# HKUST-Aerial-Robotics/FIESTA

Measured on AMD Instinct MI355X. Metric: esdf_updated_voxels_per_sec, higher is better.
Workload: dtype u32

## Files before the change

fiesta_amd/csrc/dense_map.hip:

```cpp
#include "dense_map.hpp"
#include "checkpoint.hpp"
#include "frontier_kernels.hpp"
#include "ray_query_kernels.hpp"
#include "reach_kernels.hpp"
#include "reach_path_kernels.hpp"
#include "cluster_kernels.hpp"
#include "view_kernels.hpp"
#include "ft_kernels.hpp"
#include "nn_kernels.hpp"
#include "mask_kernels.hpp"
#include "level_kernels.hpp"
#include "path_cost_kernels.hpp"
#include "path_kernels.hpp"
#include "relax_kernels.hpp"

#include <algorithm>
#include <chrono>
#include <cmath>
#include <cstdlib>
#include <cstring>

namespace fiesta {

template <typename T>
// ... 830 lines not shown
  ntiles_ = ntx_ * nty_ * ntz_;

  FIESTA_HIP_CHECK(hipStreamCreateWithFlags(&stream_, hipStreamNonBlocking));
  FIESTA_HIP_CHECK(hipEventCreate(&ev0_));
  FIESTA_HIP_CHECK(hipEventCreate(&ev1_));
  FIESTA_HIP_CHECK(hipMalloc((void **)&coc_, g.n * sizeof(vox_t)));
  FIESTA_HIP_CHECK(hipMalloc((void **)&logodds_, g.n * sizeof(double)));
  FIESTA_HIP_CHECK(hipMalloc((void **)&cnt_, g.n * sizeof(unsigned long long)));
  FIESTA_HIP_CHECK(hipMalloc((void **)&occbits_, nbitwords_ * sizeof(uint32_t)));
  FIESTA_HIP_CHECK(hipMalloc((void **)&rbits_, nbitwords_ * sizeof(uint32_t)));
  FIESTA_HIP_CHECK(hipMalloc((void **)&obsbits_, nbitwords_ * sizeof(uint32_t)));
  FIESTA_HIP_CHECK(hipMalloc((void **)&latebits_, nbitwords_ * sizeof(uint32_t)));
  FIESTA_HIP_CHECK(hipMemsetAsync(obsbits_, 0, nbitwords_ * sizeof(uint32_t), stream_));
  FIESTA_HIP_CHECK(hipMemsetAsync(latebits_, 0, nbitwords_ * sizeof(uint32_t), stream_));
  if (sharded) {
    ngoccwords_ = (int64_t)g.GX * g.GY * g.GZW;
    FIESTA_HIP_CHECK(hipMalloc((void **)&gocc_, ngoccwords_ * sizeof(uint32_t)));
    FIESTA_HIP_CHECK(hipMemsetAsync(gocc_, 0, ngoccwords_ * sizeof(uint32_t), stream_));
  }
  FIESTA_HIP_CHECK(hipMalloc((void **)&tile_epoch_, ntiles_ * sizeof(uint32_t)));
  for (int k = 0; k < 2; ++k) {
    FIESTA_HIP_CHECK(hipMalloc((void **)&cbits_[k], nbitwords_ * sizeof(uint32_t)));
    FIESTA_HIP_CHECK(hipMalloc((void **)&cstamp_[k], ntiles_ * sizeof(uint32_t)));
    FIESTA_HIP_CHECK(hipMemsetAsync(cbits_[k], 0, nbitwords_ * sizeof(uint32_t), stream_));
    FIESTA_HIP_CHECK(hipMemsetAsync(cstamp_[k], 0, ntiles_ * sizeof(uint32_t), stream_));
  }
  for (int k = 0; k < 2; ++k) {
    FIESTA_HIP_CHECK(hipMalloc((void **)&tile_flag_[k], ntiles_ * sizeof(uint32_t)));
    FIESTA_HIP_CHECK(hipMalloc((void **)&tile_list_[k], ntiles_ * sizeof(uint32_t)));
    FIESTA_HIP_CHECK(hipMemsetAsync(tile_flag_[k], 0, ntiles_ * sizeof(uint32_t), stream_));
  }
  FIESTA_HIP_CHECK(hipMalloc((void **)&counters_, C_COUNT * sizeof(unsigned long long)));
  FIESTA_HIP_CHECK(hipHostMalloc((void **)&h_counters_, C_COUNT * sizeof(unsigned long long)));
  FIESTA_HIP_CHECK(hipMemsetAsync(counters_, 0, C_COUNT * sizeof(unsigned long long), stream_));
  hipLaunchKernelGGL(k_fill<vox_t>, dim3(grid_for(g.n, 256, 4096)), dim3(256), 0, stream_, coc_, kUnobserved, g.n);
  FIESTA_HIP_CHECK(hipGetLastError());
  FIESTA_HIP_CHECK(hipMemsetAsync(logodds_, 0, g.n * sizeof(double), stream_));
  FIESTA_HIP_CHECK(hipMemsetAsync(cnt_, 0, g.n * sizeof(unsigned long long), stream_));
  FIESTA_HIP_CHECK(hipMemsetAsync(occbits_, 0, nbitwords_ * sizeof(uint32_t), stream_));
  FIESTA_HIP_CHECK(hipMemsetAsync(rbits_, 0, nbitwords_ * sizeof(uint32_t), stream_));
  FIESTA_HIP_CHECK(hipMemsetAsync(tile_epoch_, 0, ntiles_ * sizeof(uint32_t), stream_));
  set_original_range();
  pp_ = ProbParams{0, 0, 0, 0, 0};
#ifdef FIESTA_HIP_TUNING
  if (const char *e = getenv("FIESTA_HIP_PROF")) prof_ = atoi(e);
  if (const char *e = getenv("FIESTA_HIP_SPATIAL")) spatial_ = atoi(e);
  if (const char *e = getenv("FIESTA_HIP_LIST_THRESHOLD")) list_threshold_ = std::max(0, atoi(e));
  if (const char *e = getenv("FIESTA_HIP_SMALL_UPDATE")) small_update_ = std::max(0, atoi(e));
  if (const char *e = getenv("FIESTA_HIP_BOUND_SCAN")) bound_scan_ = atoi(e);
  if (const char *e = getenv("FIESTA_HIP_BLOCKS")) spatial_blocks_ = std::max(8, atoi(e) / 8 * 8);
  if (const char *e = getenv("FIESTA_HIP_BULK_RATIO")) bulk_ratio_ = atof(e);
  if (const char *e = getenv("FIESTA_HIP_FT_S0")) ft_s0_ = atoi(e);
#endif
  if (ft_s0_ != 16 && ft_s0_ != 32) throw Error(FIESTA_HIP_ERR_INVALID, "FIESTA_HIP_FT_S0 must be 16 or 32");
  for (auto &e : ft_ev_) FIESTA_HIP_CHECK(hipEventCreate(&e));
  FIESTA_HIP_CHECK(hipStreamSynchronize(stream_));
}

DenseMap::~DenseMap() {
  (void)hipSetDevice(device_);
  if (stream_) (void)hipStreamSynchronize(stream_);
  free_raycast_state();
  void *ptrs[] = {coc_,          logodds_,      cnt_,          occbits_,      rbits_,     tile_epoch_,
                  tile_flag_[0], tile_flag_[1], tile_list_[0], tile_list_[1], counters_,  cbits_[0],
                  cbits_[1],     cstamp_[0],    cstamp_[1],    gocc_,         obsbits_,   latebits_,
                  mask_ctr_};
  for (void *p : ptrs)
    if (p) (void)hipFree(p);
  if (h_counters_) (void)hipHostFree(h_counters_);
  if (h_mask_ctr_) (void)hipHostFree(h_mask_ctr_);
  delete bricks_;
  delete lv_;
  for (hipEvent_t e : evpool_) (void)hipEventDestroy(e);
  for (hipEvent_t e : ft_ev_)
    if (e) (void)hipEventDestroy(e);
  if (ev0_) (void)hipEventDestroy(ev0_);
  if (ev1_) (void)hipEventDestroy(ev1_);
  if (stream_) (void)hipStreamDestroy(stream_);
}

void DenseMap::set_prob_params(double p_hit, double p_miss, double p_min, double p_max, double p_occ) {
  auto logit = [](double x) { return std::log(x / (1 - x)); };
  pp_.l_hit = logit(p_hit);
  pp_.l_miss = logit(p_miss);
  pp_.l_min = logit(p_min);
  pp_.l_max = logit(p_max);
  pp_.l_occ = logit(p_occ);
}

void DenseMap::set_original_range() {
  Geom &g = g_;
  g.wx0 = g.wy0 = g.wz0 = 0;
  g.wx1 = g.nx - 1;
  g.wy1 = g.ny - 1;
  g.wz1 = g.nz - 1;
  g.px0 = g.wx0, g.py0 = g.wy0, g.pz0 = g.wz0;
  g.px1 = g.wx1, g.py1 = g.wy1, g.pz1 = g.wz1;
}

void DenseMap::set_update_range(const double *mn, const double *mx, bool new_vec) {
  Geom &g = g_;
  double a[3], b[3];
  for (int i = 0; i < 3; ++i) {
    a[i] = std::max(mn[i], g.lo[i]);
    b[i] = std::min(mx[i], g.hi[i]);
  }
// ... 459 lines not shown
  a.ticket = &counters_[C_FUSE_TICKET];
  if (!g.sharded && !a.g.big()) {
    a.fail_cap = (uint32_t)std::min<int64_t>(std::max<int64_t>(ncells / 64, 16), 4096);
    nn_fail_list_.ensure((size_t)a.fail_cap, stream_);
    a.fail_list = nn_fail_list_.p, a.nfail = &counters_[C_NN_BRUTE];
    if (publish && !incremental) a.nsparse = &counters_[C_NN_SPARSE];
  }
  const unsigned close_blocks = nn_last_brute_ > 0 ? (unsigned)std::min<long long>(nn_last_brute_ + 8, 512) : 1u;
  a.cursor = &counters_[C_NN_CURSOR], a.failed = &counters_[C_NN_FAILED], a.entries = &counters_[C_NN_ENTRIES];
  const bool want_max = (track_ && !tr_out_) || open_side;
  a.maxd2 = want_max ? &counters_[C_FT_MAXD2] : nullptr;
  ft_in_place_ = !g.sharded || (!open_side && alone_in_group_);
  if (!ft_in_place_) ft_out_.ensure_exact((size_t)g.n, stream_);
  a.coc = tr_out_ ? tr_out_ : ft_in_place_ ? coc_ : ft_out_.p;
  if (publish) {
    a.pub = h_counters_, a.queues = &counters_[C_INSERT], a.track_dst = track_ ? &counters_[C_MAXD2] : nullptr;
    a.tag = ++nn_tag_;
    a.pub_failed = C_NN_FAILED, a.pub_entries = C_NN_ENTRIES, a.pub_maxd2 = C_FT_MAXD2, a.pub_tag = C_NN_CURSOR, a.pub_dirty = C_NN_DIRTY;
    a.pub_brute = C_NN_BRUTE, a.pub_sparse = C_NN_SPARSE;
  }
  if (!ft_counters_clean_)
    FIESTA_HIP_CHECK(hipMemsetAsync(&counters_[C_FT_OVF0], 0, 7 * sizeof(unsigned long long), stream_));
  ft_counters_clean_ = false;
  FIESTA_HIP_CHECK(hipEventRecord(ft_ev_[0], stream_));
  if (a.szb % 4 == 0) hipLaunchKernelGGL(k_nn_cells<true>, dim3((unsigned)((nrows + 15) / 16)), dim3(1024), 0, stream_, a);
  else hipLaunchKernelGGL(k_nn_cells<false>, dim3((unsigned)((nrows + 15) / 16)), dim3(1024), 0, stream_, a);
  FIESTA_HIP_CHECK(hipGetLastError());
  FIESTA_HIP_CHECK(hipEventRecord(ft_ev_[1], stream_));
  const int lcx = a.g.lx1 - a.g.lx0, lcy = a.g.ly1 - a.g.ly0, lcz = a.g.lz1 - a.g.lz0;
  if (incremental) {
    hipLaunchKernelGGL(k_nn_mark, dim3((unsigned)std::min<unsigned long long>((ni + nd) * 3375 / 1024 + 1, 256)), dim3(1024), 0, stream_, a);
    const unsigned est = (unsigned)std::min<unsigned long long>((ni + nd) * 200 + 256, (unsigned long long)ncells / 2);
    hipLaunchKernelGGL(k_nn_lists_dirty, dim3(std::min(std::max(est / 16u, 64u), 8192u)), dim3(256), 0, stream_, a);
    FIESTA_HIP_CHECK(hipGetLastError());
    FIESTA_HIP_CHECK(hipEventRecord(ft_ev_[2], stream_));
    if (want_max) hipLaunchKernelGGL(k_nn_fill_dirty<true>, dim3(std::min(std::max(est / 4u, 64u), 8192u)), dim3(256), 0, stream_, a);
    else hipLaunchKernelGGL(k_nn_fill_dirty<false>, dim3(std::min(std::max(est / 4u, 64u), 8192u)), dim3(256), 0, stream_, a);
    FIESTA_HIP_CHECK(hipGetLastError());
    FIESTA_HIP_CHECK(hipEventRecord(ft_ev_[3], stream_));
    if (publish) {
      NnArgs c = a;
      c.nfail = nullptr, c.nsparse = nullptr;
      hipLaunchKernelGGL(k_nn_close, dim3(1), dim3(256), 0, stream_, c);
      FIESTA_HIP_CHECK(hipGetLastError());
    }
    if (st) {
      st->bulk = 1;
      st->cells = 1;
      st->nn_incremental = 1;
      st->relax_launches = 4;
    }
    return true;
  }
  if (a.g.big()) hipLaunchKernelGGL(k_nn_lists<true>, dim3((lcz + 63) / 64, (lcy + 3) / 4, lcx), dim3(1024), 0, stream_, a);
  else hipLaunchKernelGGL(k_nn_lists<false>, dim3((lcz + 63) / 64, (lcy + 3) / 4, lcx), dim3(1024), 0, stream_, a);
  FIESTA_HIP_CHECK(hipGetLastError());
  FIESTA_HIP_CHECK(hipEventRecord(ft_ev_[2], stream_));
  const int64_t nq = nrows * ((a.g.ncz + 3) / 4);
  unsigned fill_blocks = 0;
  bool full = (a.g.fx | a.g.fy | a.g.fz) == 0 && a.g.nx == g.nx && a.g.ny == g.ny && a.g.nz == g.nz && g.nx % nn::kB == 0 &&
              g.ny % nn::kB == 0 && g.nz % (4 * nn::kB) == 0;
  if (full) {
    unsigned b = (unsigned)std::min<int64_t>(nq / 4, kFillBlocks);
    while (b >= 64 && nq % (4 * (int64_t)b) != 0) --b;
    if (b >= 64) fill_blocks = b; else full = false;
  }
  const dim3 cell_grid((lcz + 3) / 4, lcy, lcx);
  const bool pairs = !full && (a.g.az % 2) == 0 && (a.g.fz % 2) == 0;
  const int64_t nq_off = (int64_t)lcx * lcy * ((lcz + 3) / 4);
  const unsigned off_blocks = (unsigned)std::max<int64_t>(1, std::min<int64_t>(kFillBlocks, (nq_off + 15) / 16));
  if (want_max) {
    if (full) hipLaunchKernelGGL((k_nn_fill_full<true>), dim3(fill_blocks), dim3(256), 0, stream_, a);
    else if (pairs) hipLaunchKernelGGL((k_nn_fill_full<true, true>), dim3(off_blocks), dim3(256), 0, stream_, a);
    else hipLaunchKernelGGL((k_nn_fill<true>), cell_grid, dim3(256), 0, stream_, a);
  } else {
    if (full) hipLaunchKernelGGL((k_nn_fill_full<false>), dim3(fill_blocks), dim3(256), 0, stream_, a);
    else if (pairs) hipLaunchKernelGGL((k_nn_fill_full<false, true>), dim3(off_blocks), dim3(256), 0, stream_, a);
    else hipLaunchKernelGGL((k_nn_fill<false>), cell_grid, dim3(256), 0, stream_, a);
  }
  FIESTA_HIP_CHECK(hipGetLastError());
  FIESTA_HIP_CHECK(hipEventRecord(ft_ev_[3], stream_));
  if (publish || a.nfail) {
    hipLaunchKernelGGL(k_nn_close, dim3(close_blocks), dim3(256), 0, stream_, a);
    FIESTA_HIP_CHECK(hipGetLastError());
  }
  if (track_ && !publish && !tr_out_)
    FIESTA_HIP_CHECK(hipMemcpyAsync(&counters_[C_MAXD2], &counters_[C_FT_MAXD2], sizeof(unsigned long long), hipMemcpyDeviceToDevice, stream_));
  if (st) {
    st->bulk = 1;
    st->cells = 1;
    st->relax_launches = 3;
  }
  return true;
}

bool DenseMap::bulk_eligible(unsigned long long ni, unsigned long long nd) {
  const Geom &g = g_;
  if (update_engine_ == 1 || update_engine_ == 3) return false;
  if (!g.full_window()) return false;
  const long long owned = (long long)(g.ox1 - g.ox0 + 1) * (g.oy1 - g.oy0 + 1) * (g.oz1 - g.oz0 + 1);
  if ((long long)h_counters_[C_OBSERVED] != owned) return false;
  if (win_dirty_) return false;
  if (stale_inf_) {
    zero_counter(C_SCRATCH);
    hipLaunchKernelGGL(k_count_stale, dim3(grid_for(g_.n, 256, 4096)), dim3(256), 0, stream_, g_, (const vox_t *)coc_,
                       &counters_[C_SCRATCH]);
    FIESTA_HIP_CHECK(hipGetLastError());
// ... 1294 lines not shown
```

fiesta_amd/csrc/dense_map.hpp:

```cpp
#pragma once
#include <algorithm>
#include <chrono>
#include <vector>

#include "../../include/fiesta_hip.h"
#include "common.hpp"

namespace fiesta {

template <typename T>
struct DevBuf {
  T *p = nullptr;
  size_t cap = 0;
  ~DevBuf() { release(); }
  void release() {
    if (p) (void)hipFree(p);
    p = nullptr;
    cap = 0;
  }
  void ensure_exact(size_t n, hipStream_t s) {
    if (n <= cap) return;
    if (p) {
      FIESTA_HIP_CHECK(hipStreamSynchronize(s));
      (void)hipFree(p);
// ... 266 lines not shown
  hipStream_t stream_ = nullptr;
  hipEvent_t ev0_ = nullptr, ev1_ = nullptr;
  std::vector<hipEvent_t> evpool_;
  hipEvent_t pool_event(size_t i);

  vox_t *coc_ = nullptr;
  double *logodds_ = nullptr;
  unsigned long long *cnt_ = nullptr;
  uint32_t *occbits_ = nullptr;
  uint32_t *rbits_ = nullptr;
  uint32_t *obsbits_ = nullptr;
  uint32_t *latebits_ = nullptr;
  uint32_t *gocc_ = nullptr;
  int64_t ngoccwords_ = 0;
  int64_t nbitwords_ = 0;

  static constexpr int tx_ = 16, ty_ = 16;
  int ntx_ = 0, nty_ = 0, ntz_ = 0, ntiles_ = 0;
  uint32_t *tile_epoch_ = nullptr;
  int update_engine_ = 0;
  LevelEngine *lv_ = nullptr;
  double bulk_ratio_ = -1;
  bool stale_inf_ = false;
  bool win_dirty_ = false;
  DevBuf<uint32_t> effocc_, mask_out_, mask_ubits_, mask_uq_, mask_qstamp_, cellnb_;
  DevBuf<unsigned long long> cellst_;
  DevBuf<unsigned long long> mask_walks_, mask_ptab_;
  DevBuf<uint8_t> cellobs_, celldist_;
  unsigned long long *mask_ctr_ = nullptr, *h_mask_ctr_ = nullptr;
  uint32_t mask_serial_ = 0;
  uint32_t notes_ = 0;
  long long mask_obs_count_ = -1;
  size_t mask_seg_cap_ = 0;
  int mask_chain_hint_ = 10;
  const uint32_t *tr_occ_ = nullptr;
  vox_t *tr_out_ = nullptr;
  const uint8_t *tr_cellobs_ = nullptr;
  int ft_s0_ = 16;
  static constexpr int kFtBlocks = 1024;
  double ft_last_ms_ = 0;
  bool ft_in_place_ = true;
  bool alone_in_group_ = true;
  bool queues_zeroed_ = false;
  bool ft_counters_clean_ = false;
  DevBuf<uint32_t> ft_inter_, ft_out_;
  DevBuf<uint32_t> nn_ctab_, nn_sites_, nn_lists_, nn_dirty_flag_, nn_dirty_list_, nn_fail_list_;
  long long nn_last_brute_ = 0;
  bool nn_valid_ = false;
  double nn_last_ms_ = 0;
  long long nn_last_nocc_ = -1;
  bool nn_clean_ = false;
  unsigned long long nn_tag_ = 1ull << 40;
  bool tried_cells_ = false;
  int nn_fail_streak_ = 0, nn_skip_ = 0;
  DevBuf<unsigned long long> ft_spill_;
  DevBuf<uint16_t> ft_rowlist_;
  DevBuf<int32_t> ft_rowcnt_;
  hipEvent_t ft_ev_[4] = {nullptr, nullptr, nullptr, nullptr};
  uint32_t *cbits_[2] = {nullptr, nullptr};
  uint32_t *cstamp_[2] = {nullptr, nullptr};
  int prof_ = 0;
  int spatial_blocks_ = 1024;
  bool track_ = false;
  int bound_scan_ = 1;
  static constexpr uint32_t kCountOnDevice = 0xFFFFFFFFu;
  int chain_hint_ = 4;
  hipEvent_t last_chain_event_ = nullptr;
  bool h_counters_fresh_ = false;
  int small_update_ = 4096;
  int list_threshold_ = 1024;
  int spatial_ = 1;
  uint32_t serial_ = 0;
  uint32_t *tile_flag_[2] = {nullptr, nullptr};
  uint32_t *tile_list_[2] = {nullptr, nullptr};
  uint32_t epoch_ = 0;

  DevBuf<uint32_t> touched_, ins_, del_;
  int64_t touched_upper_ = 0;
  unsigned long long host_counts_[4] = {0, 0, 0, 0};
  bool host_counts_valid_ = false;
  unsigned long long *counters_ = nullptr;
  unsigned long long *h_counters_ = nullptr;

  DevBuf<unsigned char> stage_a_, stage_b_, stage_c_;
  PlannerScratch planner_;
  struct RaycastState;
  RaycastState *rc_ = nullptr;
  void free_raycast_state();
  friend struct RaycastAccess;

  Snapshot snaps_[4];

  static constexpr int64_t kHostQueries = 8;
  struct HostBricks;
  struct HostWords;
  HostBricks *bricks_ = nullptr;
  uint64_t field_epoch_ = 1;
  const uint32_t *host_brick(int x, int y, int z);
  int host_occ(int x, int y, int z);
};

}
```

fiesta_amd/csrc/nn_core.hpp:

```cpp
#pragma once
#include <stdint.h>

#if defined(__HIPCC__)
#define FIESTA_NN_HD __host__ __device__
#else
#define FIESTA_NN_HD
#include <math.h>
#endif
#if defined(__HIP_DEVICE_COMPILE__)
#define FIESTA_NN_MUL(a, b) __mul24((a), (b))
#define FIESTA_NN_SQRT(x) __builtin_amdgcn_sqrtf(x)
#else
#define FIESTA_NN_MUL(a, b) ((a) * (b))
#define FIESTA_NN_SQRT(x) sqrtf(x)
#endif

namespace fiesta {
namespace nn {

constexpr int kB = 8;
constexpr int kCap = 30;
constexpr int kSH = 9;
constexpr int kBias = 3 * 7 * 7;
constexpr int kKfirst = 1;
constexpr int kKmax = 7;
constexpr int kStride = 128;
constexpr int kRaw = 32;
constexpr int kThin = 16;
constexpr uint32_t kPadK = 0xFFFFFFFFu;
constexpr int kWhySparse = 1, kWhyDense = 2, kWhyOpen = 3;
constexpr int kNone = 0x7FFFFFFF;

struct Geom {
  int nx, ny, nz;
  int ncx, ncy, ncz;
  int wx, wy, wz;
  int open;
  int lx0, lx1, ly0, ly1, lz0, lz1;
  int fx, fy, fz;
  int ax, ay, az;
  FIESTA_NN_HD inline bool big() const { return nx > 1024 || ny > 1024 || nz > 1024; }
};
FIESTA_NN_HD inline Geom whole_geom(int nx, int ny, int nz) {
  Geom g{};
  g.nx = nx, g.ny = ny, g.nz = nz;
  g.ncx = (nx + kB - 1) / kB, g.ncy = (ny + kB - 1) / kB, g.ncz = (nz + kB - 1) / kB;
  g.lx1 = g.ncx, g.ly1 = g.ncy, g.lz1 = g.ncz;
  g.ax = nx, g.ay = ny, g.az = nz;
  return g;
}
constexpr int kRegionMax = 1536;
FIESTA_NN_HD inline bool region_geom(const int *G, const int *l0, const int *ln, int mc, Geom &g, int *rlo) {
  int n[3], f[3], c0[3], c1[3], open = 0;
  for (int k = 0; k < 3; ++k) {
    int lo = l0[k] - mc;
    lo = (lo < 0 ? 0 : lo) & ~((k == 2 ? 32 : kB) - 1);
    int hi = (l0[k] + ln[k] + mc + kB - 1) & ~(kB - 1);
    if (hi > G[k]) hi = G[k];
    rlo[k] = lo, n[k] = hi - lo, f[k] = l0[k] - lo;
    if (lo > 0) open |= 1 << (2 * k);
    if (hi < G[k]) open |= 2 << (2 * k);
    c0[k] = f[k] / kB, c1[k] = (f[k] + ln[k] - 1) / kB + 1;
    if (n[k] > kRegionMax) return false;
  }
  g = whole_geom(n[0], n[1], n[2]);
  g.wx = rlo[0], g.wy = rlo[1], g.wz = rlo[2];
  g.open = open;
// ... 198 lines not shown
        }
        if (keep) {
          const int k = team.slot();
          if (k < kRaw) team.put(k, pack_p(px, py, pz));
        }
      }
    }
    raw = team.count();
    if (kfirst >= 2) break;
  }
  int n = 0;
  if (raw > 0 && raw <= kRaw) {
    if (raw > kThin) {
      for (int k = team.rank; k < raw; k += Team::lanes) {
        const uint32_t pk = team.get(k);
        int px, py, pz;
        unpack_p(pk, px, py, pz);
        bool dead = false;
        for (int j = 0; j < raw && !dead; ++j) {
          int qx, qy, qz;
          unpack_p(team.get(j) & 0xFFFFFFu, qx, qy, qz);
          dead = j != k && dominated(px, py, pz, qx, qy, qz, qx * qx + qy * qy + qz * qz);
        }
        if (dead) team.put(k, pk | 0x80000000u);
      }
    }
    team.restart();
    for (int k = team.rank; k < raw; k += Team::lanes) {
      const uint32_t pk = team.get(k);
      if (pk & 0x80000000u) continue;
      int px, py, pz;
      unpack_p(pk, px, py, pz);
      const int i = team.slot();
      if (i < kCap) {
        uint32_t *e = out + 4 + 4 * i;
        e[0] = entry_b(py, pz), e[1] = entry_k(px, py, pz, i), e[2] = entry_m(px);
        e[3] = (((uint32_t)(px + ox + fr.wx) & 1023u) << 20) | (((uint32_t)(py + oy + fr.wy) & 1023u) << 10) | ((uint32_t)(pz + oz + fr.wz) & 1023u);
      }
    }
    n = team.count();
  }
  if (n > kCap) n = 0;
  if (team.rank == 0) {
    out[0] = (uint32_t)n;
    out[1] = n ? (uint32_t)reach : ((uint32_t)kKmax | ((uint32_t)why << 8) | ((uint32_t)reach << 16));
    if (n & 1) {
      uint32_t *e = out + 4 + 4 * n;
      e[0] = 0u, e[1] = kPadK, e[2] = 0u, e[3] = 0u;
    }
  }
  return n;
}

}
}
```

fiesta_amd/csrc/nn_kernels.hpp:

```cpp
#pragma once
#include "common.hpp"
#include "nn_core.hpp"

namespace fiesta {

struct NnArgs {
  nn::Geom g;
  const uint8_t *cellobs;
  const uint32_t *occ;
  int sx0, sy0, szb;
  int sny, snzw;
  uint32_t *ctab;
  uint32_t *sites;
  uint32_t sites_cap;
  uint32_t *lists;
  unsigned long long *cursor;
  unsigned long long *failed;
  unsigned long long *entries;
  unsigned long long *maxd2;
  vox_t *coc;
  uint32_t *dump;
  unsigned long long *pub, *queues, *track_dst;
  unsigned long long tag;
  int pub_failed, pub_entries, pub_maxd2, pub_tag, pub_dirty, pub_brute, pub_sparse;
// ... 303 lines not shown
      s_te2[team_i] = (uint32_t)te2, s_tw[team_i] = tw, s_key[team_i] = (uint8_t)key;
      atomicAdd(&s_bin[key], 1u);
    }
  }
  __syncthreads();
  if (tid == 0) {
    uint32_t at = 0;
    for (int k = 0; k < 8; ++k) {
      const uint32_t c = s_bin[k];
      s_bin[k] = at, at += c;
    }
  }
  __syncthreads();
  if (tid < 256) s_order[atomicAdd(&s_bin[s_key[tid]], 1u)] = (uint16_t)tid;
  __syncthreads();
  const int ci = s_order[team_i];
  const int cz = cz0 + (ci & 63), cy = cy0 + (ci >> 6);
  int n = 0;
  bool live = cz < g.lz1 && cy < g.ly1;
  if (live && a.cellobs && a.cellobs[((int64_t)cx * g.ncy + cy) * g.ncz + cz] == 0) {
    live = false;
    if (team.rank == 0) a.lists[(((int64_t)cx * g.ncy + cy) * g.ncz + cz) * nn::kStride] = 0u;
  }
  if (live) {
    const int64_t cell = ((int64_t)cx * g.ncy + cy) * g.ncz + cz;
    uint32_t *rec = a.lists + cell * nn::kStride;
    n = -1;
    if (staged) n = nn::build_list(ssrc, team, cx, cy, cz, rec, true, (int)s_te2[ci], s_tw[ci], fr);
    if (n < 0) {
      const HybridSrcT<WRAP> src{ssrc, nn::PlainSrcT<WRAP>{a.ctab, a.sites, g.ncx, g.ncy, g.ncz}, X0, Y0, Zf};
      n = nn::build_list(src, team, cx, cy, cz, rec, false, nn::kNone, 0xFFFFFFFFu, fr);
    }
  }
  bool hard = live && team.rank == 0 && n == 0;
  if (hard && a.fail_list && fr.open == 0 && *a.nfail < a.fail_cap) {
    const unsigned long long at = atomicAdd(a.nfail, 1ull);
    if (at < a.fail_cap) {
      a.fail_list[at] = (uint32_t)(((int64_t)cx * g.ncy + cy) * g.ncz + cz);
      hard = false;
    }
  }
  const unsigned long long bad = __ballot(hard);
  int sum = (live && team.rank == 0) ? n : 0;
  for (int off = 32; off > 0; off >>= 1) sum += __shfl_xor(sum, off);
  if ((tid & 63) == 0) {
    if (bad) atomicAdd(&s_bad, (uint32_t)__popcll(bad));
    if (sum) atomicAdd(&s_sum, (uint32_t)sum);
    __threadfence_block();
    if (atomicAdd(&s_done, 1u) == 15u) {
      const uint32_t b = atomicAdd(&s_bad, 0u), t = atomicAdd(&s_sum, 0u);
      if (b) atomicAdd(a.failed, (unsigned long long)b);
      if (t) atomicAdd(a.entries, (unsigned long long)t);
    }
  }
}

__device__ __forceinline__ void nn_dot4_pair(uint32_t a, uint32_t b0, uint32_t b1, int &d0, int &d1) {
  asm("v_dot4_i32_i8 %0, %2, %3, 0\n\tv_dot4_i32_i8 %1, %2, %4, 0\n\ts_nop 2" : "=&v"(d0), "=&v"(d1) : "v"(a), "v"(b0), "v"(b1));
}

#ifndef FIESTA_FILL_BLOCKS
#define FIESTA_FILL_BLOCKS 16384
#endif
constexpr int kFillBlocks = FIESTA_FILL_BLOCKS;
constexpr int kListPad = 256;

template <bool TRACK, bool OFFSET = false>
__global__ __launch_bounds__(256) void k_nn_fill_full(NnArgs a) {
  constexpr int kTileRow = 40;
  __shared__ __attribute__((aligned(16))) uint32_t land[4][2][nn::kStride];
  __shared__ __attribute__((aligned(16))) uint32_t tile[4][nn::kB * kTileRow];
  const nn::Geom &g = a.g;
  if (*a.failed) return;
  const int lane = threadIdx.x & 63, wave = __builtin_amdgcn_readfirstlane((int)(threadIdx.x >> 6));
  const int quads = OFFSET ? (g.lz1 - g.lz0 + 3) >> 2 : g.ncz >> 2;
  const int rows_y = OFFSET ? g.ly1 - g.ly0 : g.ncy;
  const uint32_t nq = (uint32_t)((OFFSET ? g.lx1 - g.lx0 : g.ncx) * rows_y) * (uint32_t)quads;
  const uint32_t per = OFFSET ? (nq + gridDim.x * 4u - 1u) / (gridDim.x * 4u) : nq / (gridDim.x * 4u);
  const uint32_t q0 = (blockIdx.x * 4u + (uint32_t)wave) * per, q1 = OFFSET ? min(q0 + per, nq) : q0 + per;
  if (OFFSET && q0 >= q1) return;
  const int row0 = (int)(q0 / (uint32_t)quads);
  const int y = lane >> 3, z = lane & 7;
  const uint32_t ayz = (uint32_t)y | ((uint32_t)z << 8);
  const int64_t plane = (int64_t)g.ny * g.nz;
  const int loff4 = y * g.nz + 4 * z;
  uint32_t dmax = 0;
  const uint32_t zone0 = (uint32_t)(size_t)&land[wave][0][0];
  uint32_t *const mytile = &tile[wave][0];
  struct At { int cx, cy, q; };
  auto fetch = [&](const At &c, const int cell_of_quad, const int zone) {
    const int64_t cell = OFFSET ? ((int64_t)(g.lx0 + c.cx) * g.ncy + (g.ly0 + c.cy)) * g.ncz + min(g.lz0 + 4 * c.q + cell_of_quad, g.lz1 - 1)
                                : ((int64_t)c.cx * g.ncy + c.cy) * g.ncz + 4 * c.q + cell_of_quad;
    const uint32_t *lp = a.lists + cell * nn::kStride + lane, *hp = lp + 64;
    const uint32_t at = zone0 + (uint32_t)zone * (uint32_t)(nn::kStride * 4);
    asm volatile("s_mov_b32 m0, %0\n\tglobal_load_lds_dword %1, off\n\t"
                 "s_mov_b32 m0, %2\n\tglobal_load_lds_dword %3, off"
                 : : "s"(at), "v"(lp), "s"(at + 256u), "v"(hp) : "memory", "m0");
  };
  auto advance = [&](At &c) {
    if (++c.q == quads) {
      c.q = 0;
      if (++c.cy == rows_y) c.cy = 0, ++c.cx;
    }
  };
  auto serve = [&](const int zone, uint32_t *ww, const bool col_in, const int xin_lo, const int xin_hi) {
    const uint32_t *lz = &land[wave][zone][0];
// ... 345 lines not shown
```

Measured before the change: 7.991 billion.

## Build NN candidate lists per block of cells with shared gather

Adds a new k_nn_lists_blocks kernel that handles a 16- or 32-voxel block of cells together. It finds the block's nearest site, gathers the candidate sites once into shared memory, prunes them with a box-dominance test, and then derives per-cell lists from that shared subset, including a sub-block level for the 32 case. The goal is to avoid each cell re-reading and re-filtering overlapping neighbourhoods, at the cost of more shared memory, extra block-wide syncs, and an overflow fallback that marks cells as failed. It is on by default for non-sharded, closed, small geometries and can be turned off with an environment variable.

```diff
diff --git a/fiesta_amd/csrc/dense_map.hip b/fiesta_amd/csrc/dense_map.hip
--- a/fiesta_amd/csrc/dense_map.hip
+++ b/fiesta_amd/csrc/dense_map.hip
@@ -906,6 +906,11 @@
   if (const char *e = getenv("FIESTA_HIP_BULK_RATIO")) bulk_ratio_ = atof(e);
   if (const char *e = getenv("FIESTA_HIP_FT_S0")) ft_s0_ = atoi(e);
 #endif
+  if (const char *e = getenv("FIESTA_NN_LISTS")) {
+    if (strcmp(e, "cells") == 0) nn_list_blocks_ = 0;
+    else if (strcmp(e, "blocks") == 0) nn_list_blocks_ = 1;
+    else throw Error(FIESTA_HIP_ERR_INVALID, "FIESTA_NN_LISTS must be cells or blocks");
+  }
   if (ft_s0_ != 16 && ft_s0_ != 32) throw Error(FIESTA_HIP_ERR_INVALID, "FIESTA_HIP_FT_S0 must be 16 or 32");
   for (auto &e : ft_ev_) FIESTA_HIP_CHECK(hipEventCreate(&e));
   FIESTA_HIP_CHECK(hipStreamSynchronize(stream_));
@@ -1471,7 +1476,12 @@
     }
     return true;
   }
-  if (a.g.big()) hipLaunchKernelGGL(k_nn_lists<true>, dim3((lcz + 63) / 64, (lcy + 3) / 4, lcx), dim3(1024), 0, stream_, a);
+  if (nn_list_blocks_ && !g.sharded && a.g.open == 0 && !a.g.big()) {
+    if (nn::block_edge_for((long long)h_counters_[C_NOCC], (long long)g.n) == 32)
+      hipLaunchKernelGGL(k_nn_lists_blocks<32>, dim3((a.g.ncz + 3) / 4, (a.g.ncy + 3) / 4, (a.g.ncx + 3) / 4), dim3(256), 0, stream_, a);
+    else
+      hipLaunchKernelGGL(k_nn_lists_blocks<16>, dim3((a.g.ncz + 1) / 2, (a.g.ncy + 1) / 2, (a.g.ncx + 1) / 2), dim3(64), 0, stream_, a);
+  } else if (a.g.big()) hipLaunchKernelGGL(k_nn_lists<true>, dim3((lcz + 63) / 64, (lcy + 3) / 4, lcx), dim3(1024), 0, stream_, a);
   else hipLaunchKernelGGL(k_nn_lists<false>, dim3((lcz + 63) / 64, (lcy + 3) / 4, lcx), dim3(1024), 0, stream_, a);
   FIESTA_HIP_CHECK(hipGetLastError());
   FIESTA_HIP_CHECK(hipEventRecord(ft_ev_[2], stream_));
diff --git a/fiesta_amd/csrc/dense_map.hpp b/fiesta_amd/csrc/dense_map.hpp
--- a/fiesta_amd/csrc/dense_map.hpp
+++ b/fiesta_amd/csrc/dense_map.hpp
@@ -342,6 +342,7 @@
   bool nn_clean_ = false;
   unsigned long long nn_tag_ = 1ull << 40;
   bool tried_cells_ = false;
+  int nn_list_blocks_ = 1;
   int nn_fail_streak_ = 0, nn_skip_ = 0;
   DevBuf<unsigned long long> ft_spill_;
   DevBuf<uint16_t> ft_rowlist_;
diff --git a/fiesta_amd/csrc/nn_core.hpp b/fiesta_amd/csrc/nn_core.hpp
--- a/fiesta_amd/csrc/nn_core.hpp
+++ b/fiesta_amd/csrc/nn_core.hpp
@@ -10,9 +10,11 @@
 #if defined(__HIP_DEVICE_COMPILE__)
 #define FIESTA_NN_MUL(a, b) __mul24((a), (b))
 #define FIESTA_NN_SQRT(x) __builtin_amdgcn_sqrtf(x)
+#define FIESTA_NN_DIV(a, b) ((int)(((float)(a) + 0.5f) * __builtin_amdgcn_rcpf((float)(b))))
 #else
 #define FIESTA_NN_MUL(a, b) ((a) * (b))
 #define FIESTA_NN_SQRT(x) sqrtf(x)
+#define FIESTA_NN_DIV(a, b) ((a) / (b))
 #endif
 
 namespace fiesta {
@@ -317,5 +319,204 @@
   return n;
 }
 
-}
-}
+constexpr int kRawB = 64;
+template <int B>
+struct BlockCaps;
+template <>
+struct BlockCaps<32> {
+  static constexpr int gather = 4096, list = 1024, sub = 256;
+};
+template <>
+struct BlockCaps<16> {
+  static constexpr int gather = 2048, list = 512, sub = 512;
+};
+FIESTA_NN_HD inline int block_edge_for(long long nocc, long long nvox) { return nocc * 1000 <= nvox ? 32 : 16; }
+
+template <int B>
+FIESTA_NN_HD inline int box_e2(int px, int py, int pz) {
+  const int ex = 2 * px - (B - 1), ey = 2 * py - (B - 1), ez = 2 * pz - (B - 1);
+  return FIESTA_NN_MUL(ex, ex) + FIESTA_NN_MUL(ey, ey) + FIESTA_NN_MUL(ez, ez);
+}
+template <int B>
+FIESTA_NN_HD inline int box_rad2(int e2) {
+  const float r = FIESTA_NN_SQRT((float)e2) + (2.0f * (B - 1) * 1.7320508f + 0.04f);
+  return (int)(r * r) + 1;
+}
+template <int B>
+FIESTA_NN_HD inline int box_gap(int d) { return d ? 16 * d + (B - 15) : 0; }
+template <int B>
+FIESTA_NN_HD inline int box_cells(float r2) {
+  const int m = (int)((r2 + (float)(15 - B) + 0.02f) * 0.0625f);
+  return m < 0 ? 0 : m;
+}
+template <int B>
+FIESTA_NN_HD inline int box_reach(int rad2) { return box_cells<B>(FIESTA_NN_SQRT((float)rad2)); }
+template <int B>
+FIESTA_NN_HD inline bool box_dominated(int px, int py, int pz, int qx, int qy, int qz, int q2) {
+  const int ax = px - qx, ay = py - qy, az = pz - qz;
+  return FIESTA_NN_MUL(px, px) + FIESTA_NN_MUL(py, py) + FIESTA_NN_MUL(pz, pz) - q2 >=
+         FIESTA_NN_MUL(2 * (B - 1), (ax > 0 ? ax : 0) + (ay > 0 ? ay : 0) + (az > 0 ? az : 0));
+}
+template <int B>
+FIESTA_NN_HD inline int box_window_reach(int e2, int qx, int qy, int qz) {
+  if (e2 == kNone) return kKmax + 1;
+  const int fx = qx > B - 1 - qx ? qx : B - 1 - qx, fy = qy > B - 1 - qy ? qy : B - 1 - qy, fz = qz > B - 1 - qz ? qz : B - 1 - qz;
+  const int Kc = ((int)(FIESTA_NN_SQRT((float)(FIESTA_NN_MUL(fx, fx) + FIESTA_NN_MUL(fy, fy) + FIESTA_NN_MUL(fz, fz))) + 0.02f) + 7) >> 3;
+  const int Kb = box_reach<B>(box_rad2<B>(e2));
+  return Kb < Kc ? Kb : Kc;
+}
+
+template <int B>
+FIESTA_NN_HD inline bool box_row(int r, int K, int rad2, int &rx, int &ry, int &m) {
+  constexpr int NB = B / kB;
+  const int E = NB + 2 * K, rq = FIESTA_NN_DIV(r, E);
+  rx = rq - K, ry = r - FIESTA_NN_MUL(rq, E) - K;
+  const int gx = box_gap<B>(rx < 0 ? -rx : rx >= NB ? rx - NB + 1 : 0), gy = box_gap<B>(ry < 0 ? -ry : ry >= NB ? ry - NB + 1 : 0);
+  const int rem = rad2 - FIESTA_NN_MUL(gx, gx) - FIESTA_NN_MUL(gy, gy);
+  if (rem < 0) return false;
+  m = box_cells<B>(FIESTA_NN_SQRT((float)rem));
+  m = m > K ? K : m;
+  return true;
+}
+
+struct SoloGroup {
+  static constexpr int lanes = 1;
+  int rank = 0;
+  FIESTA_NN_HD inline void nearest(int &, uint32_t &) const {}
+  FIESTA_NN_HD inline int place(bool keep, int &count) const {
+    const int at = count;
+    count += keep ? 1 : 0;
+    return at;
+  }
+  FIESTA_NN_HD inline void sync() const {}
+};
+
+template <int B, class Group>
+FIESTA_NN_HD inline void flat_nearest(const Group &grp, const uint32_t *cand, int n, int ox, int oy, int oz, int &e2, uint32_t &w) {
+  e2 = kNone, w = 0xFFFFFFFFu;
+  for (int i = grp.rank; i < n; i += Group::lanes) {
+    const uint32_t c = cand[i];
+    int px, py, pz;
+    site_offset<false>(c, ox, oy, oz, px, py, pz);
+    const int e = box_e2<B>(px, py, pz);
+    if (e < e2 || (e == e2 && c < w)) e2 = e, w = c;
+  }
+  grp.nearest(e2, w);
+}
+template <int B, class Group>
+FIESTA_NN_HD inline int flat_keep(const Group &grp, const uint32_t *cand, int n, int ox, int oy, int oz, uint32_t tw, uint32_t *out, int cap) {
+  int qx, qy, qz;
+  site_offset<false>(tw, ox, oy, oz, qx, qy, qz);
+  const int q2 = FIESTA_NN_MUL(qx, qx) + FIESTA_NN_MUL(qy, qy) + FIESTA_NN_MUL(qz, qz);
+  int count = 0;
+  for (int base = 0; base < n; base += Group::lanes) {
+    const int i = base + grp.rank;
+    bool keep = false;
+    uint32_t c = 0;
+    if (i < n) {
+      c = cand[i];
+      int px, py, pz;
+      site_offset<false>(c, ox, oy, oz, px, py, pz);
+      keep = c == tw || !box_dominated<B>(px, py, pz, qx, qy, qz, q2);
+    }
+    const int at = grp.place(keep, count);
+    if (keep && at < cap) out[at] = c;
+  }
+  return count;
+}
+template <class Group>
+FIESTA_NN_HD inline int flat_keep_cell(const Group &grp, const uint32_t *cand, int n, int cx, int cy, int cz, uint32_t tw, int Kw, uint32_t *raw) {
+  const int ox = kB * cx, oy = kB * cy, oz = kB * cz;
+  int qx, qy, qz;
+  site_offset<false>(tw, ox, oy, oz, qx, qy, qz);
+  const int q2 = FIESTA_NN_MUL(qx, qx) + FIESTA_NN_MUL(qy, qy) + FIESTA_NN_MUL(qz, qz);
+  const int lo = -kB * Kw, hi = kB * Kw + kB - 1;
+  int count = 0;
+  for (int base = 0; base < n; base += Group::lanes) {
+    const int i = base + grp.rank;
+    bool keep = false;
+    int px = 0, py = 0, pz = 0;
+    if (i < n) {
+      const uint32_t c = cand[i];
+      site_offset<false>(c, ox, oy, oz, px, py, pz);
+      const bool in = px >= lo && px <= hi && py >= lo && py <= hi && pz >= lo && pz <= hi;
+      keep = in && (c == tw || !dominated(px, py, pz, qx, qy, qz, q2));
+    }
+    const int at = grp.place(keep, count);
+    if (keep && at < kRawB) raw[at] = pack_p(px, py, pz);
+  }
+  return count;
+}
+template <class Group>
+FIESTA_NN_HD inline void flat_thin(const Group &grp, uint32_t *raw, int n) {
+  for (int idx = grp.rank; idx < n * n; idx += Group::lanes) {
+    const int k = FIESTA_NN_DIV(idx, n), j = idx - FIESTA_NN_MUL(k, n);
+    if (j == k) continue;
+    const uint32_t pk = raw[k] & 0xFFFFFFu;
+    int px, py, pz, qx, qy, qz;
+    unpack_p(pk, px, py, pz);
+    unpack_p(raw[j] & 0xFFFFFFu, qx, qy, qz);
+    if (dominated(px, py, pz, qx, qy, qz, FIESTA_NN_MUL(qx, qx) + FIESTA_NN_MUL(qy, qy) + FIESTA_NN_MUL(qz, qz))) raw[k] = pk | 0x80000000u;
+  }
+  grp.sync();
+}
+template <class Group>
+FIESTA_NN_HD inline int flat_entries(const Group &grp, const uint32_t *raw, int n, int cx, int cy, int cz, const Frame &fr, uint32_t *out) {
+  const int ox = kB * cx, oy = kB * cy, oz = kB * cz;
+  int count = 0;
+  for (int base = 0; base < n; base += Group::lanes) {
+    const int k = base + grp.rank;
+    const uint32_t pk = k < n ? raw[k] : 0x80000000u;
+    const bool keep = !(pk & 0x80000000u);
+    const int i = grp.place(keep, count);
+    if (keep && i < kCap) {
+      int px, py, pz;
+      unpack_p(pk, px, py, pz);
+      uint32_t *e = out + 4 + 4 * i;
+      e[0] = entry_b(py, pz), e[1] = entry_k(px, py, pz, i), e[2] = entry_m(px);
+      e[3] = (((uint32_t)(px + ox + fr.wx) & 1023u) << 20) | (((uint32_t)(py + oy + fr.wy) & 1023u) << 10) | ((uint32_t)(pz + oz + fr.wz) & 1023u);
+    }
+  }
+  return count > kCap ? 0 : count;
+}
+FIESTA_NN_HD inline void record_head(uint32_t *out, int n, int reach, int why) {
+  out[0] = (uint32_t)n;
+  out[1] = n ? (uint32_t)reach : ((uint32_t)kKmax | ((uint32_t)why << 8) | ((uint32_t)reach << 16));
+  if (n & 1) {
+    uint32_t *e = out + 4 + 4 * n;
+    e[0] = 0u, e[1] = kPadK, e[2] = 0u, e[3] = 0u;
+  }
+}
+struct CellHead {
+  int reach, why, raw_n;
+  FIESTA_NN_HD inline bool thin() const { return raw_n > kThin && raw_n <= kRawB; }
+};
+template <class Group>
+FIESTA_NN_HD inline CellHead flat_cell_keep(const Group &grp, const uint32_t *cand, int n, int cx, int cy, int cz, uint32_t *raw) {
+  int te2;
+  uint32_t tw;
+  flat_nearest<kB>(grp, cand, n, kB * cx, kB * cy, kB * cz, te2, tw);
+  CellHead h{kKmax, kWhySparse, 0};
+  const int Kw = window_reach<false>(te2, tw, cx, cy, cz);
+  if (Kw <= kKmax) {
+    h.reach = Kw, h.why = kWhyDense;
+    h.raw_n = flat_keep_cell(grp, cand, n, cx, cy, cz, tw, Kw, raw);
+    grp.sync();
+  }
+  return h;
+}
+template <class Group>
+FIESTA_NN_HD inline int flat_cell_record(const Group &grp, const uint32_t *raw, const CellHead &h, int cx, int cy, int cz, const Frame &fr, uint32_t *out) {
+  const int cnt = h.raw_n <= kRawB ? flat_entries(grp, raw, h.raw_n, cx, cy, cz, fr, out) : 0;
+  if (grp.rank == 0) record_head(out, cnt, h.reach, h.why);
+  return cnt;
+}
+template <class Group>
+FIESTA_NN_HD inline int flat_cell(const Group &grp, const uint32_t *cand, int n, int cx, int cy, int cz, const Frame &fr, uint32_t *raw, uint32_t *out) {
+  const CellHead h = flat_cell_keep(grp, cand, n, cx, cy, cz, raw);
+  if (h.thin()) flat_thin(grp, raw, h.raw_n);
+  return flat_cell_record(grp, raw, h, cx, cy, cz, fr, out);
+}
+
+}
+}
diff --git a/fiesta_amd/csrc/nn_kernels.hpp b/fiesta_amd/csrc/nn_kernels.hpp
--- a/fiesta_amd/csrc/nn_kernels.hpp
+++ b/fiesta_amd/csrc/nn_kernels.hpp
@@ -379,6 +379,225 @@
       if (b) atomicAdd(a.failed, (unsigned long long)b);
       if (t) atomicAdd(a.entries, (unsigned long long)t);
     }
+  }
+}
+
+template <int N>
+struct LaneGroup {
+  static constexpr int lanes = N;
+  int rank;
+  unsigned long long below, all;
+  __device__ __forceinline__ LaneGroup(int lane) : rank(lane & (N - 1)) {
+    all = (N == 64 ? ~0ull : ((1ull << (N & 63)) - 1ull) << (lane & ~(N - 1)));
+    below = all & ((1ull << lane) - 1ull);
+  }
+  __device__ __forceinline__ void nearest(int &e2, uint32_t &w) const {
+#pragma unroll
+    for (int off = 1; off < N; off <<= 1) {
+      const int oe = __shfl_xor(e2, off);
+      const uint32_t ow = (uint32_t)__shfl_xor((int)w, off);
+      if (oe < e2 || (oe == e2 && ow < w)) e2 = oe, w = ow;
+    }
+  }
+  __device__ __forceinline__ int place(bool keep, int &count) const {
+    const unsigned long long bits = __ballot(keep);
+    const int at = count + __popcll(bits & below);
+    count += __popcll(bits & all);
+    return at;
+  }
+  __device__ __forceinline__ void sync() const { __builtin_amdgcn_fence(__ATOMIC_ACQ_REL, "wavefront"); }
+};
+template <int T>
+struct BlockGroup {
+  static constexpr int lanes = T;
+  int rank;
+  __device__ __forceinline__ void sync() const {}
+};
+
+template <int B>
+__global__ __launch_bounds__(B == 32 ? 256 : 64) void k_nn_lists_blocks(NnArgs a) {
+  typedef nn::BlockCaps<B> Caps;
+  constexpr int NB = B / nn::kB, CELLS = NB * NB * NB, T = B == 32 ? 256 : 64, W = T / 64, LPC = T / CELLS;
+  constexpr int NR = (NB + 2 * nn::kKmax) * (NB + 2 * nn::kKmax);
+  constexpr int kRawStride = nn::kRawB + 1;
+  constexpr int kScratch = Caps::gather > CELLS * kRawStride ? Caps::gather : CELLS * kRawStride;
+  __shared__ uint32_t s_sites[kScratch];
+  __shared__ uint32_t s_list[Caps::list];
+  __shared__ uint32_t s_sub[B == 32 ? 8 * Caps::sub : 1];
+  __shared__ uint32_t s_rfirst[NR], s_roff[NR];
+  __shared__ uint16_t s_rcnt[NR];
+  __shared__ int s_re2[W];
+  __shared__ uint32_t s_rw[W], s_wcnt[W], s_subn[8];
+  __shared__ uint32_t s_total, s_ovf, s_bad, s_sum, s_nthin;
+  __shared__ uint16_t s_thin[CELLS];
+  const nn::Geom &g = a.g;
+  if (*a.failed) return;
+  const int tid = (int)threadIdx.x, lane = tid & 63, wave = tid >> 6;
+  const int cx0 = NB * (int)blockIdx.z, cy0 = NB * (int)blockIdx.y, cz0 = NB * (int)blockIdx.x;
+  const int ox = nn::kB * cx0, oy = nn::kB * cy0, oz = nn::kB * cz0;
+  const nn::PlainSrc src{a.ctab, a.sites, g.ncx, g.ncy, g.ncz};
+  const nn::Frame fr = nn::frame_of(g);
+  if (tid == 0) s_ovf = 0, s_bad = 0, s_sum = 0, s_nthin = 0;
+  int te2 = nn::kNone;
+  uint32_t tw = 0xFFFFFFFFu;
+  for (int K = 0; K <= nn::kKmax && te2 == nn::kNone; ++K) {
+    const int E = NB + 2 * K;
+    for (int idx = tid; idx < E * E * 4; idx += T) {
+      const int row = idx >> 2, rq = FIESTA_NN_DIV(row, E);
+      uint32_t i, i1;
+      src.bounds(cx0 + rq - K, cy0 + row - rq * E - K, cz0 - K, cz0 + NB - 1 + K, i, i1);
+      for (i += (uint32_t)(idx & 3); i < i1; i += 4) {
+        const uint32_t w = a.sites[i];
+        int px, py, pz;
+        nn::site_offset<false>(w, ox, oy, oz, px, py, pz);
+        const int e = nn::box_e2<B>(px, py, pz);
+        if (e < te2 || (e == te2 && w < tw)) te2 = e, tw = w;
+      }
+    }
+    LaneGroup<64>(lane).nearest(te2, tw);
+    if (W > 1) {
+      if (lane == 0) s_re2[wave] = te2, s_rw[wave] = tw;
+      __syncthreads();
+#pragma unroll
+      for (int w = 0; w < W; ++w) {
+        const int oe = s_re2[w];
+        const uint32_t ow = s_rw[w];
+        if (oe < te2 || (oe == te2 && ow < tw)) te2 = oe, tw = ow;
+      }
+      __syncthreads();
+    }
+  }
+  int K = 0, rad2 = 0, nrows = 0;
+  if (te2 != nn::kNone) {
+    int qx, qy, qz;
+    nn::site_offset<false>(tw, ox, oy, oz, qx, qy, qz);
+    rad2 = nn::box_rad2<B>(te2);
+    K = min(nn::box_window_reach<B>(te2, qx, qy, qz), nn::kKmax);
+    nrows = (NB + 2 * K) * (NB + 2 * K);
+  }
+  for (int r = tid; r < nrows; r += T) {
+    int rx, ry, m;
+    uint32_t i = 0, i1 = 0;
+    if (nn::box_row<B>(r, K, rad2, rx, ry, m)) src.bounds(cx0 + rx, cy0 + ry, cz0 - m, cz0 + NB - 1 + m, i, i1);
+    s_rfirst[r] = i, s_rcnt[r] = (uint16_t)min(i1 - i, 65535u);
+  }
+  __syncthreads();
+  if (wave == 0) {
+    uint32_t base = 0;
+    for (int r0 = 0; r0 < nrows; r0 += 64) {
+      const int r = r0 + lane;
+      const uint32_t c = r < nrows ? (uint32_t)s_rcnt[r] : 0u;
+      uint32_t incl = c;
+      for (int off = 1; off < 64; off <<= 1) {
+        const uint32_t up = (uint32_t)__shfl_up((int)incl, off);
+        if (lane >= off) incl += up;
+      }
+      if (r < nrows) s_roff[r] = base + incl - c;
+      base += (uint32_t)__shfl((int)incl, 63);
+    }
+    if (lane == 0) {
+      s_total = base;
+      if (base > (uint32_t)Caps::gather) s_ovf = 1;
+    }
+  }
+  __syncthreads();
+  const int ng = (int)s_total;
+  bool ovf = s_ovf != 0;
+  if (!ovf)
+    for (int k = tid; k < ng; k += T) {
+      int lo = 0, hi = nrows - 1;
+      while (lo < hi) {
+        const int mid = (lo + hi + 1) >> 1;
+        if (s_roff[mid] <= (uint32_t)k) lo = mid; else hi = mid - 1;
+      }
+      s_sites[k] = a.sites[s_rfirst[lo] + ((uint32_t)k - s_roff[lo])];
+    }
+  __syncthreads();
+  const LaneGroup<64> wg(lane);
+  int nl = 0;
+  if (!ovf) {
+    if (W == 1) {
+      nl = nn::flat_keep<B>(wg, s_sites, ng, ox, oy, oz, tw, s_list, Caps::list);
+    } else {
+      const int seg = ((ng + W - 1) / W + 63) & ~63;
+      const int start = min(wave * seg, ng), len = min(seg, ng - start);
+      const int mine = nn::flat_keep<B>(wg, s_sites + start, len, ox, oy, oz, tw, s_sites + start, len);
+      if (lane == 0) s_wcnt[wave] = (uint32_t)mine;
+      __syncthreads();
+      int off = 0;
+#pragma unroll
+      for (int w = 0; w < W; ++w) {
+        const int c = (int)s_wcnt[w];
+        if (w < wave) off += c;
+        nl += c;
+      }
+      if (nl <= Caps::list)
+        for (int i = lane; i < mine; i += 64) s_list[off + i] = s_sites[start + i];
+    }
+    ovf = nl > Caps::list;
+  }
+  __syncthreads();
+  if (B == 32) {
+    if (!ovf) {
+#pragma unroll
+      for (int h = 0; h < 2; ++h) {
+        const int s = 2 * wave + h;
+        const int sox = ox + 16 * ((s >> 2) & 1), soy = oy + 16 * ((s >> 1) & 1), soz = oz + 16 * (s & 1);
+        int se2;
+        uint32_t sw;
+        nn::flat_nearest<16>(wg, s_list, nl, sox, soy, soz, se2, sw);
+        const int ns = nn::flat_keep<16>(wg, s_list, nl, sox, soy, soz, sw, s_sub + s * Caps::sub, Caps::sub);
+        if (lane == 0) s_subn[s] = (uint32_t)ns;
+      }
+    }
+    __syncthreads();
+  }
+  const int ci = tid / LPC;
+  const LaneGroup<LPC> cg(lane);
+  const int sb = B == 32 ? ci >> 3 : 0, cc = ci & 7;
+  const int cx = cx0 + (B == 32 ? 2 * ((sb >> 2) & 1) : 0) + ((cc >> 2) & 1), cy = cy0 + (B == 32 ? 2 * ((sb >> 1) & 1) : 0) + ((cc >> 1) & 1),
+            cz = cz0 + (B == 32 ? 2 * (sb & 1) : 0) + (cc & 1);
+  const int64_t cell = ((int64_t)cx * g.ncy + cy) * g.ncz + cz;
+  bool live = cx < g.lx1 && cy < g.ly1 && cz < g.lz1;
+  if (live && a.cellobs && a.cellobs[cell] == 0) {
+    live = false;
+    if (cg.rank == 0) a.lists[cell * nn::kStride] = 0u;
+  }
+  uint32_t *const rec = a.lists + (live ? cell : 0) * nn::kStride;
+  uint32_t *const raw = s_sites + ci * kRawStride;
+  nn::CellHead head{nn::kKmax, nn::kWhySparse, 0};
+  if (live && !ovf) {
+    const bool sub_ok = B == 32 && s_subn[sb] <= (uint32_t)Caps::sub;
+    head = nn::flat_cell_keep(cg, sub_ok ? s_sub + sb * Caps::sub : s_list, sub_ok ? (int)s_subn[sb] : nl, cx, cy, cz, raw);
+    if (head.thin() && cg.rank == 0) s_thin[atomicAdd(&s_nthin, 1u)] = (uint16_t)(ci | (head.raw_n << 8));
+  }
+  __syncthreads();
+  for (uint32_t q = 0; q < s_nthin; ++q) {
+    const int c = s_thin[q] & 255, n = s_thin[q] >> 8;
+    nn::flat_thin(BlockGroup<T>{tid}, s_sites + c * kRawStride, n);
+  }
+  __syncthreads();
+  int n = 0;
+  if (live) n = nn::flat_cell_record(cg, raw, head, cx, cy, cz, fr, rec);
+  bool hard = live && cg.rank == 0 && n == 0;
+  if (hard && a.fail_list && fr.open == 0 && *a.nfail < a.fail_cap) {
+    const unsigned long long at = atomicAdd(a.nfail, 1ull);
+    if (at < a.fail_cap) {
+      a.fail_list[at] = (uint32_t)cell;
+      hard = false;
+    }
+  }
+  const unsigned long long bad = __ballot(hard);
+  int sum = (live && cg.rank == 0) ? n : 0;
+  for (int off = 32; off > 0; off >>= 1) sum += __shfl_xor(sum, off);
+  if (lane == 0) {
+    if (bad) atomicAdd(&s_bad, (uint32_t)__popcll(bad));
+    if (sum) atomicAdd(&s_sum, (uint32_t)sum);
+  }
+  __syncthreads();
+  if (tid == 0) {
+    if (s_bad) atomicAdd(a.failed, (unsigned long long)s_bad);
+    if (s_sum) atomicAdd(a.entries, (unsigned long long)s_sum);
   }
 }
 
```

Result: no change. 7.973 billion (-0.2%).
